# jcasal-homer/HomerHEVC

Measured on AMD Instinct MI355X. Metric: encoded frames/sec, 1080p & 2160p YUV420 fixed-QP IPPP, 1/2/4/8 MI355X, higher is better.
Workload: dtype int16; 1 GPU; cfg2-1080p-encode; sequences_per_gpu=256, width=1920, height=1080, wfpp_num_threads=17, qp=32, gop=IPPP intra_period=100

## Files before the change

homerhevc_amd/csrc/enc/enc_common.h:

```cpp
#pragma once
#include "enc_prims.h"
#if !defined(__HIPCC__)
#include <stdio.h>
#include <stdlib.h>
#endif

#if !defined(__HIPCC__) && defined(HENC_TRACE_ENABLE)
#include <stdio.h>
extern "C" FILE *henc_trace_file;
#define HENC_TRACE(...) do { if (henc_trace_file) fprintf(henc_trace_file, __VA_ARGS__); } while (0)
#define HENC_TRACE_PW(e, tag)                                                                                                                      \
	do {                                                                                                                                       \
		if (henc_trace_file) {                                                                                                             \
			unsigned a_[3] = {0, 0, 0};                                                                                                \
			for (int c_ = 0; c_ < 3; c_++) {                                                                                           \
				const int n_ = c_ ? 32 : 64;                                                                                       \
				const pred_t *p_ = c_ ? (e).w->pred_c[c_ - 1] : (e).w->pred_y;                                                     \
				for (int y_ = 0; y_ < n_; y_++)                                                                                    \
					for (int x_ = 0; x_ < n_; x_++) a_[c_] += (unsigned)(p_[y_ * n_ + x_] & 0xffff) * (unsigned)(1 + ((x_ + 3 * y_) & 7)); \
			}                                                                                                                          \
			fprintf(henc_trace_file, "PW %s ctu=%d pred=%u,%u,%u\n", tag, (e).ctu->ctu_number, a_[0], a_[1], a_[2]);                   \
		}                                                                                                                                  \
	} while (0)
#else
#define HENC_TRACE(...) do { } while (0)
#define HENC_TRACE_PW(e, tag) do { } while (0)
#endif

enum { PF_SETUP = 0, PF_MERGE, PF_ME_INT, PF_ME_SUB, PF_PRED_INTER, PF_ENC_INTER, PF_INTRA_SEARCH, PF_INTRA_TU, PF_INTRA_CHROMA, PF_CONSOLIDATE, PF_WAIT, PF_TOTAL, PF_PRIM0, PF_COUNT = PF_PRIM0 + 2 * PP_COUNT + 2 };
#if defined(__HIPCC__) && defined(HENC_PROFILE)
#define HENC_PROF_T0() const unsigned long long prof_t0_ = __builtin_amdgcn_s_memtime()
#if defined(HENC_QPROF)
#define HENC_PROF_ADD(e, cat) do { if ((cat) == PF_TOTAL && (e).prof && threadIdx.x == 0) (e).prof[cat] += __builtin_amdgcn_s_memtime() - prof_t0_; } while (0)
#define HENC_QPROF_T0() unsigned long long qprof_t_ = __builtin_amdgcn_s_memtime()
#define HENC_QPROF_MARK(e, cat) do { const unsigned long long now_ = __builtin_amdgcn_s_memtime(); if ((e).prof && threadIdx.x == 0) (e).prof[cat] += now_ - qprof_t_; qprof_t_ = now_; } while (0)
#define HENC_QPROF_ARG , unsigned long long &qprof_t_
#define HENC_QPROF_PASS , qprof_t_
#else
#define HENC_PROF_ADD(e, cat) do { if ((e).prof && threadIdx.x == 0) (e).prof[cat] += __builtin_amdgcn_s_memtime() - prof_t0_; } while (0)
#endif
#else
#define HENC_PROF_T0() do { } while (0)
#define HENC_PROF_ADD(e, cat) do { } while (0)
#endif
#if !defined(HENC_QPROF_MARK)
#define HENC_QPROF_T0() do { } while (0)
#define HENC_QPROF_MARK(e, cat) do { } while (0)
#define HENC_QPROF_ARG
#define HENC_QPROF_PASS
#endif

namespace henc {

#if defined(__HIPCC__)
extern __constant__ Geo henc_geo_table[NNODES];
#endif
#if defined(__HIP_DEVICE_COMPILE__)
struct GeoTable {
	const Geo *p;
	__device__ __forceinline__ const Geo &operator[](int i) const { return henc_geo_table[__builtin_amdgcn_readfirstlane(i)]; }
	__device__ __forceinline__ const Geo &lane(int i) const { return henc_geo_table[i]; }
};
#else
struct GeoTable {
	const Geo *p;
	HENC_INLINE const Geo &operator[](int i) const { return p[i]; }
	HENC_INLINE const Geo &lane(int i) const { return p[i]; }
};
#endif

constexpr int NHELP_MAX = 3;
constexpr int NODES_RESIDENT = 21, NODES_D3 = 85, NODE_QUAD_D3 = 16, NODE_QUAD_D4 = 64, NODE_SLOTS = NODES_RESIDENT + NODE_QUAD_D3 + NODE_QUAD_D4;
HENC_INLINE int node_quadrant(int idx) { return idx < NODES_D3 ? (idx - NODES_RESIDENT) >> 4 : (idx - NODES_D3) >> 6; }
HENC_INLINE int node_slot(int idx)
{
	return idx < NODES_RESIDENT ? idx : (idx < NODES_D3 ? NODES_RESIDENT + ((idx - NODES_RESIDENT) & (NODE_QUAD_D3 - 1)) : NODES_RESIDENT + NODE_QUAD_D3 + ((idx - NODES_D3) & (NODE_QUAD_D4 - 1)));
}
constexpr int NHELP_ = 1
#if defined(HENC_NHELP)
	+ (HENC_NHELP) - 1
#endif
	;
constexpr int HSCRATCH_ELEMS = 2048 + 144;
constexpr int LDS_OFF_WORK = 0, LDS_OFF_NODES = (int)((sizeof(Work) + 15) & ~(size_t)15), LDS_OFF_SEQ = LDS_OFF_NODES + (int)((sizeof(Node) * NODE_SLOTS + 15) & ~(size_t)15) + NHELP_ * HSCRATCH_ELEMS * 2,
	      LDS_OFF_FRAME = LDS_OFF_SEQ + (int)((sizeof(Seq) + 15) & ~(size_t)15), LDS_OFF_BOX = LDS_OFF_SEQ + (int)((sizeof(Seq) + sizeof(FrameCtx) + 31) & ~(size_t)15);
#if defined(__HIP_DEVICE_COMPILE__)
#define HENC_AT(T, OFFSET) LdsAt<T, OFFSET>
#else
#define HENC_AT(T, OFFSET) FastPtr<T>
#endif

constexpr int LDS_BOX_BYTES = 160, LDS_ENC_BYTES = 272;
constexpr int LDS_OFF_ENC = LDS_OFF_BOX + LDS_BOX_BYTES;
constexpr int LDS_OFF_RD = LDS_OFF_ENC + (1 + NHELP_) * LDS_ENC_BYTES;
struct Enc {
	unsigned long long *prof;
	HENC_AT(const Seq, LDS_OFF_SEQ) seq;
	HENC_AT(const FrameCtx, LDS_OFF_FRAME) f;
	const DevTables *T;
	FastPtr<const FastTables> ft;
	GeoTable geo;
	CtuInfo *ctus;
	CtuPublic *ctu;
// ... 450 lines not shown
```

homerhevc_amd/csrc/enc/enc_inter.h:

```cpp
#pragma once
#include "enc_common.h"

namespace henc {

#if !defined(__HIPCC__)
template <class G>
HENC_HD void mc_luma_interp(const G g, Enc &__restrict__ e, const int16_t *ref, int rs, int16_t *pred, int ps, int n, int mvx, int mvy)
{
	HENC_ENC_IN_LDS(e);
	const int xf = mvx & 3, yf = mvy & 3;
	const int16_t *src = ref + (mvy >> 2) * rs + (mvx >> 2);
	if (xf == 0) interp_stage<8>(g, src, rs, pred, ps, yf, n, n, 1, 1, 1);
	else if (yf == 0) interp_stage<8>(g, src, rs, pred, ps, xf, n, n, 0, 1, 1);
	else {
		int16_t *tmp = e.mc_tmp_y;
		const int ts = e.mc_tmp_y_stride;
		interp_stage<8>(g, src - 3 * rs, rs, tmp, ts, xf, n, n + 7, 0, 1, 0);
		interp_stage<8>(g, tmp + 3 * ts, ts, pred, ps, yf, n, n, 1, 0, 1);
	}
}
template <class G>
HENC_HD void mc_chroma_interp(const G g, Enc &__restrict__ e, const int16_t *ref, int rs, int16_t *pred, int ps, int n, int mvx, int mvy)
{
	HENC_ENC_IN_LDS(e);
// ... 86 lines not shown
}
template <int N>
HENC_INLINE uint32_t pick(const uint32_t (&a)[N], int idx)
{
#if defined(__HIP_DEVICE_COMPILE__)
	uint32_t v[N];
#pragma unroll
	for (int k = 0; k < N; k++) { v[k] = a[k]; asm("" : "+s"(v[k])); }
	uint32_t r = v[0];
#pragma unroll
	for (int k = 1; k < N; k++) r = idx == k ? v[k] : r;
	return r;
#else
	uint32_t r = a[0];
	for (int k = 1; k < N; k++) r = idx == k ? a[k] : r;
	return r;
#endif
}

HENC_INLINE uint32_t mv_cost_fast(const MvCandList &l, double corr, int mvx, int mvy, int *best_idx)
{
	uint32_t best = 0x7fffffff;
	int bi = 0;
	for (int i = 0; i < l.num; i++) {
		const double cx = corr * ((float)habs(l.mv[i].x - mvx)), cy = corr * ((float)habs(l.mv[i].y - mvy));
		const uint32_t c = (uint32_t)(cx + cy + .5);
		if (best > c) { best = c; bi = i; }
	}
	*best_idx = bi;
	return best;
}
HENC_INLINE float bit_sqrt(float x)
{
	union { float f; uint32_t u; } v;
	v.f = x;
	v.u += 127u << 23;
	v.u >>= 1;
	return v.f;
}
HENC_INLINE uint32_t mv_cost_sqrt(const MvCandList &l, uint32_t qp, int mvx, int mvy, int *best_idx)
{
	uint32_t best = 0x7fffffff;
	int bi = 0;
	for (int i = 0; i < l.num; i++) {
		const double cx = (float)qp * bit_sqrt((float)habs(l.mv[i].x - mvx));
		const double cy = (float)qp * bit_sqrt((float)habs(l.mv[i].y - mvy));
		const uint32_t c = (uint32_t)(3. + cx + cy + .5);
		if (best > c) { best = c; bi = i; }
	}
	*best_idx = bi;
	return best;
}

template <class G>
HENC_HD uint32_t motion_estimation(const G g, Enc &__restrict__ e, int ox, int oy, int gx, int gy, int size, const MvCandList &amvp, const MvCandList &search, double corr,
				   int action, MV *mv_io, MV *subpix_out)
{
	HENC_ENC_IN_LDS(e);
	static constexpr int ds[4][2] = {{-1, 0}, {0, -1}, {1, 0}, {0, 1}};
	static constexpr int db[8][2] = {{-2, 0}, {-1, -1}, {0, -2}, {1, -1}, {2, 0}, {1, 1}, {0, 2}, {-1, 1}};
	static constexpr int ref_h[9][2] = {{0, 0}, {0, -1}, {0, 1}, {-1, 0}, {1, 0}, {-1, -1}, {1, -1}, {-1, 1}, {1, 1}};
	static constexpr int ref_q[9][2] = {{0, 0}, {0, -1}, {0, 1}, {-1, -1}, {1, -1}, {-1, 0}, {1, 0}, {-1, 1}, {1, 1}};
	const int fw = e.seq->width, fh = e.seq->height;
	const int xlow = (gx - SEARCH_RANGE_X) < 0 ? -gx : -SEARCH_RANGE_X, xhigh = (gx + SEARCH_RANGE_X) > (fw - size) ? fw - gx - size : SEARCH_RANGE_X;
	const int ylow = (gy - SEARCH_RANGE_Y) < 0 ? -gy : -SEARCH_RANGE_Y, yhigh = (gy + SEARCH_RANGE_Y) > (fh - size) ? fh - gy - size : SEARCH_RANGE_Y;
	uint32_t cur_sad = 0, cur_rd = 0, best_sad = 0xffffffffu;
	int cur_x = 0, cur_y = 0, best_x = 0, best_y = 0, mvx = 0, mvy = 0, subx = 0, suby = 0, dummy;
#define HENC_IN_WIN(x, y) ((x) >= xlow && (x) <= xhigh && (y) >= ylow && (y) <= yhigh)
#define HENC_TRY(x, y, sad_, on_better)                                                            \
	do {                                                                                       \
		if (HENC_IN_WIN(x, y)) {                                                           \
			const uint32_t s_ = (sad_);                                                \
			const uint32_t rd_ = s_ + mv_cost_fast(amvp, corr, (x) << 2, (y) << 2, &dummy); \
			if (rd_ < cur_rd) { on_better; cur_sad = s_; cur_rd = rd_; cur_x = (x); cur_y = (y); } \
		}                                                                                  \
	} while (0)
	HENC_PROF_T0();
	if (action & ME_PEL) {
		bool early = false;
		cur_x = hclip(0, xlow, xhigh);
		cur_y = hclip(0, ylow, yhigh);
		{
			int qx[4], qy[4];
			bool ok[4];
			uint32_t s4[4];
			qx[0] = cur_x << 2; qy[0] = cur_y << 2; ok[0] = true;
			for (int i = 0; i < 3; i++) {
				const int x = i < search.num ? search.mv[i].x >> 2 : 0, y = i < search.num ? search.mv[i].y >> 2 : 0;
				qx[i + 1] = x << 2; qy[i + 1] = y << 2;
				ok[i + 1] = i < search.num && !(x == 0 && y == 0) && HENC_IN_WIN(x, y);
			}
			cand_sads<4>(g, e, ox, oy, gx, gy, size, qx, qy, ok, s4);
			cur_sad = s4[0];
			cur_rd = cur_sad + mv_cost_fast(amvp, corr, cur_x << 2, cur_y << 2, &dummy);
			best_sad = cur_sad; best_x = cur_x; best_y = cur_y;
			if (best_sad <= 0) early = true;
			if (!early) {
				for (int i = 0; i < search.num; i++) {
					const int x = search.mv[i].x >> 2, y = search.mv[i].y >> 2;
					if (x == 0 && y == 0) continue;
					HENC_TRY(x, y, pick(s4, i + 1), (void)0);
				}
				best_sad = cur_sad; best_x = cur_x; best_y = cur_y;
				if (best_sad <= 0) early = true;
			}
		}
// ... 46 lines not shown
				}
				cand_sads<4>(g, e, ox, oy, gx, gy, size, qx, qy, ok, s4);
				for (int i = next_start; i < next_start + search_size; i++) {
					const int idx = i % 4, x = best_x + ds[idx][0], y = best_y + ds[idx][1];
					HENC_TRY(x, y, pick(s4, idx), (next_start = (idx - 1 + 4) % 4, search_size = 3));
				}
				if (best_x == cur_x && best_y == cur_y) break;
				best_sad = cur_sad; best_x = cur_x; best_y = cur_y;
			}
		}
		best_sad = cur_sad; best_x = cur_x; best_y = cur_y;
		mvx = best_x << 2; mvy = best_y << 2;
	} else {
		mvx = mv_io->x; mvy = mv_io->y;
	}
	HENC_PROF_ADD(e, PF_ME_INT);
	if (action & ME_HALF) {
		int bidx = 0, bx = 0, by = 0;
		best_x = mvx >> 2; best_y = mvy >> 2;
		int qx[9], qy[9];
		bool ok[9];
		uint32_t sads[9];
		for (int i = 0; i < 9; i++) { qx[i] = (best_x << 2) + ref_h[i][0] * 2; qy[i] = (best_y << 2) + ref_h[i][1] * 2; ok[i] = true; }
		cand_sads<9>(g, e, ox, oy, gx, gy, size, qx, qy, ok, sads);
		if (!(action & ME_PEL)) cur_sad = sads[0];
		for (int i = 0; i < 9; i++) {
			const int cx = ref_h[i][0] * 2, cy = ref_h[i][1] * 2;
			const uint32_t s = pick(sads, i);
			if (s < cur_sad) { cur_sad = s; bx = cx; by = cy; bidx = i; }
		}
		mvx = (best_x << 2) + bx; mvy = (best_y << 2) + by; subx = bx; suby = by;
		best_sad = cur_sad;
		if (action & ME_QUARTER) {
			const int hx = ref_h[bidx][0], hy = ref_h[bidx][1];
			bx = hx * 2; by = hy * 2;
			for (int i = 0; i < 9; i++) { qx[i] = (best_x << 2) + hx * 2 + ref_q[i][0]; qy[i] = (best_y << 2) + hy * 2 + ref_q[i][1]; }
			cand_sads<9>(g, e, ox, oy, gx, gy, size, qx, qy, ok, sads);
			for (int i = 0; i < 9; i++) {
				const int cx = hx * 2 + ref_q[i][0], cy = hy * 2 + ref_q[i][1];
				const uint32_t s = pick(sads, i);
				if (s < cur_sad) { cur_sad = s; bx = cx; by = cy; }
			}
			best_sad = cur_sad;
			mvx = (best_x << 2) + bx; mvy = (best_y << 2) + by; subx = bx; suby = by;
		}
	}
#undef HENC_IN_WIN
#undef HENC_TRY
	HENC_PROF_ADD(e, PF_ME_SUB);
	mv_io->x = mvx; mv_io->y = mvy;
	subpix_out->x = subx; subpix_out->y = suby;
	return best_sad;
}

struct CornerNodes { int lb, tl, tr; };
HENC_INLINE CornerNodes corner_nodes(Enc &__restrict__ e, int ni)
{
	HENC_ENC_IN_LDS(e);
	const Geo &q = e.geo[ni];
	const int np = q.size >> 2, base = cfg_depth_start(CFG_MAX_CU_DEPTH);
	CornerNodes c;
	c.lb = base + raster2abs(q.raster_index + 16 * (np - 1));
	c.tl = base + raster2abs(q.raster_index);
	c.tr = base + raster2abs(q.raster_index + np - 1);
	return c;
}
struct NbUnit {
	int there, pred_mode, inter_mode, ref_idx;
	MV mv;
};
HENC_INLINE NbUnit nb_unit(Enc &__restrict__ e, const CtuPublic *c, uint32_t idx)
{
	HENC_ENC_IN_LDS(e);
	const CtuPublic *p = c ? c : e.ctu;
	const uint32_t i = c ? idx : 0;
	NbUnit u;
	u.pred_mode = p->pred_mode[i];
	u.inter_mode = p->inter_mode[i];
	u.ref_idx = p->mv_ref_idx[i];
	u.mv = p->mv_ref[i];
	u.there = c != nullptr;
	return u;
}
HENC_INLINE int equal_motion(const NbUnit &a, const NbUnit &b)
{
	if (a.inter_mode != b.inter_mode) return 0;
	if (a.inter_mode & 1) {
		if (a.mv.x != b.mv.x || a.mv.y != b.mv.y || a.ref_idx != b.ref_idx) return 0;
	}
	return 1;
}

HENC_INLINE int add_amvp_cand(MvCandList &l, const NbUnit &u)
{
	if (u.there && u.ref_idx >= 0) {
		l.mv[l.num++] = u.mv;
		return 1;
	}
	return 0;
}
HENC_INLINE void get_amvp_candidates(Enc &__restrict__ e, int ni, MvCandList &l)
{
	HENC_ENC_IN_LDS(e);
	const CornerNodes cn = corner_nodes(e, ni);
	uint32_t idx_lb = 0, idx_l = 0, idx_tr = 0, idx_t = 0, idx_tl = 0;
	l.num = 0;
// ... 475 lines not shown
```

homerhevc_amd/csrc/k_primtest.hip:

```cpp
#include <stdlib.h>
#include <string.h>
#include <vector>

#include "common.h"
#include "enc/enc_prims.h"

using namespace henc;

hmr_gpu_ctx *hmr_default_ctx();

namespace {

enum { PT_SAD = 1, PT_SSD, PT_PREDICT, PT_RECONST, PT_VARIANCE, PT_INTRA_PRED, PT_FILL_REFS, PT_ADI_FILTER, PT_TRANSFORM, PT_ITRANSFORM, PT_QUANT, PT_INV_QUANT };

struct PtArgs {
	int op, bytes;
	int p[12];
	long off[6];
};

int g_bytes = 0;

__global__ __launch_bounds__(64) void k_primtest(PtArgs a, int16_t *arena, uint8_t *arena8, const DevTables *T, uint32_t *ret)
{
	const WaveGrp g{(int)threadIdx.x};
	const int *p = a.p;
	auto A = [&](int k) { return arena + a.off[k]; };
	auto B = [&](int k) { return arena8 + a.off[k]; };
	uint32_t r = 0;
	switch (a.op) {
	case PT_SAD: r = blk_sad(g, A(0), p[0], A(1), p[1], p[2]); break;
	case PT_SSD: r = a.bytes ? blk_ssd(g, B(0), p[0], B(1), p[1], p[2]) : blk_ssd(g, A(0), p[0], A(1), p[1], p[2]); break;
	case PT_PREDICT:
		if (a.bytes) blk_predict(g, B(0), p[0], B(1), p[1], A(2), p[2], p[3]);
		else blk_predict(g, A(0), p[0], A(1), p[1], A(2), p[2], p[3]);
		break;
	case PT_RECONST: {
		const int16_t *res = p[1] ? A(1) : nullptr;
		if (a.bytes) blk_reconst(g, B(0), p[0], res, p[1], A(2), p[2], p[3]);
		else blk_reconst(g, A(0), p[0], res, p[1], A(2), p[2], p[3]);
		break;
	}
	case PT_VARIANCE: r = a.bytes ? blk_modified_variance(g, B(0), p[1], p[0], p[2]) : blk_modified_variance(g, A(0), p[1], p[0], p[2]); break;
	case PT_INTRA_PRED:
		if (a.bytes) {
			intra_predict(g, B(0), p[0], A(1), p[1], p[2], p[3]);
			g.sync();
			for (int i = g.tid; i < p[1] * p[1]; i += 64) A(0)[(i / p[1]) * p[0] + i % p[1]] = B(0)[(i / p[1]) * p[0] + i % p[1]];
		} else intra_predict(g, A(0), p[0], A(1), p[1], p[2], p[3]);
		break;
	case PT_FILL_REFS: intra_fill_refs(g, A(0), p[0], p[1], p[2], p[3], p[4], p[5], p[6], p[7], A(1)); break;
	case PT_ADI_FILTER: intra_adi_filter(g, A(0), A(1), p[0], p[1]); break;
	case PT_TRANSFORM:
		if (a.bytes) tr_forward(g, (const FastTables *)nullptr, T, B(0), p[0], B(3), p[0], A(1), A(2), p[1], p[2]);
		else tr_forward(g, (const FastTables *)nullptr, T, A(0), p[0], A(3), p[0], A(1), A(2), p[1], p[2]);
		break;
	case PT_ITRANSFORM: tr_inverse(g, (const FastTables *)nullptr, T, A(0), p[0], A(1), A(2), p[1], p[2]); break;
	case PT_QUANT: r = (uint32_t)quantize(g, (const FastTables *)nullptr, T, A(0), A(1), A(2), p[0], p[1], p[2], p[3], p[4], p[5], p[6], p[7], p[8]); break;
// ... 16 lines not shown
	if (!c) { fprintf(stderr, "hmr_gpu_prim_*: no device\n"); abort(); }
	PtArgs a;
	memset(&a, 0, sizeof a);
	a.op = op;
	a.bytes = g_bytes;
	for (int i = 0; i < np; i++) a.p[i] = p[i];
	size_t total = 0;
	for (int k = 0; k < nops; k++) {
		a.off[k] = (long)total;
		total += (ops[k].elems + 31) & ~(size_t)31;
	}
	std::vector<int16_t> h(total, 0);
	std::vector<uint8_t> h8(total, 0);
	for (int k = 0; k < nops; k++)
		if (ops[k].in) memcpy(h.data() + a.off[k], ops[k].in, ops[k].elems * 2);
	for (size_t i = 0; i < total; i++) h8[i] = (uint8_t)h[i];
	int16_t *d = nullptr;
	uint8_t *d8 = nullptr;
	uint32_t *dr = nullptr, r = 0;
	if (hipMalloc((void **)&d, total * 2 + 64) != hipSuccess || hipMalloc((void **)&d8, total + 64) != hipSuccess || hipMalloc((void **)&dr, 4) != hipSuccess) abort();
	(void)hipMemcpy(d, h.data(), total * 2, hipMemcpyHostToDevice);
	(void)hipMemcpy(d8, h8.data(), total, hipMemcpyHostToDevice);
	hipLaunchKernelGGL(k_primtest, dim3(1), dim3(64), 0, c->stream, a, d, d8, (const DevTables *)c->tables, dr);
	if (hipStreamSynchronize(c->stream) != hipSuccess) { fprintf(stderr, "hmr_gpu_prim_*: %s\n", hipGetErrorString(hipGetLastError())); abort(); }
	(void)hipMemcpy(h.data(), d, total * 2, hipMemcpyDeviceToHost);
	(void)hipMemcpy(&r, dr, 4, hipMemcpyDeviceToHost);
	for (int k = 0; k < nops; k++)
		if (ops[k].out) memcpy(ops[k].out, h.data() + a.off[k], ops[k].elems * 2);
	(void)hipFree(d); (void)hipFree(d8); (void)hipFree(dr);
	return r;
}

template <int MAXC>
__device__ __forceinline__ void multi_sad_all(const WaveGrp g, const uint8_t *src, const uint8_t *plane, const long long *off, int stride, int n, uint32_t *out)
{
	const uint8_t *cand[MAXC];
#pragma unroll
	for (int k = 0; k < MAXC; k++) cand[k] = off[k] < 0 ? nullptr : plane + off[k];
	uint32_t r[MAXC];
	multi_sad_u8<MAXC>(g, src, n, cand, stride, r);
	if (g.tid == 0) {
#pragma unroll
		for (int k = 0; k < MAXC; k++) out[k] = r[k];
	}
}
__global__ __launch_bounds__(64) void k_primtest_multi_sad(int maxc, const uint8_t *src, const uint8_t *plane, const long long *off, int stride, int n, uint32_t *out)
{
	const WaveGrp g{(int)threadIdx.x};
	off += (size_t)blockIdx.x * maxc;
	out += (size_t)blockIdx.x * maxc;
	if (maxc == 4) multi_sad_all<4>(g, src, plane, off, stride, n, out);
	else if (maxc == 8) multi_sad_all<8>(g, src, plane, off, stride, n, out);
	else multi_sad_all<9>(g, src, plane, off, stride, n, out);
}

size_t span(int stride, int rows, int cols) { return stride ? (size_t)stride * (rows - 1) + cols : (size_t)cols; }

}

extern "C" {

void hmr_gpu_prim_bytes(int on) { g_bytes = on ? 1 : 0; }

uint32_t hmr_gpu_prim_sad(int16_t *src, uint32_t src_stride, int16_t *pred, uint32_t pred_stride, int size)
{
	if (g_bytes) {
		std::vector<uint8_t> blk(64 * 64, 0), plane(span((int)pred_stride, size, size));
		for (int y = 0; y < size; y++)
			for (int x = 0; x < size; x++) {
				blk[y * 64 + x] = (uint8_t)src[(size_t)y * src_stride + x];
				plane[(size_t)y * pred_stride + x] = (uint8_t)pred[(size_t)y * pred_stride + x];
			}
		const int64_t off[4] = {0, -1, 0, -1};
		uint32_t out[4] = {0, 0, 0, 0};
		if (hmr_gpu_prim_multi_sad(4, blk.data(), plane.data(), plane.size(), off, 1, (int)pred_stride, size, out) != HMR_GPU_OK) { fprintf(stderr, "hmr_gpu_prim_sad: %s\n", hmr_gpu_last_error()); return 0xFFFFFFFFu; }
		if (out[1] != 0 || out[3] != 0 || out[2] != out[0]) {
			hmr_set_error("hmr_gpu_prim_sad: candidates {p, -, p, -} gave %u %u %u %u", out[0], out[1], out[2], out[3]);
			fprintf(stderr, "%s\n", hmr_gpu_last_error());
			return 0xFFFFFFFFu;
		}
		return out[0];
	}
	Operand ops[2] = {{src, nullptr, span((int)src_stride, size, size)}, {pred, nullptr, span((int)pred_stride, size, size)}};
	const int p[3] = {(int)src_stride, (int)pred_stride, size};
	return run(PT_SAD, p, 3, ops, 2);
}
uint32_t hmr_gpu_prim_ssd16b(int16_t *src, uint32_t src_stride, int16_t *pred, uint32_t pred_stride, int size)
{
	Operand ops[2] = {{src, nullptr, span((int)src_stride, size, size)}, {pred, nullptr, span((int)pred_stride, size, size)}};
	const int p[3] = {(int)src_stride, (int)pred_stride, size};
	return run(PT_SSD, p, 3, ops, 2);
}
void hmr_gpu_prim_predict(int16_t *orig, int orig_stride, int16_t *pred, int pred_stride, int16_t *residual, int residual_stride, int size)
{
	Operand ops[3] = {{orig, nullptr, span(orig_stride, size, size)}, {pred, nullptr, span(pred_stride, size, size)}, {residual, residual, span(residual_stride, size, size)}};
	const int p[4] = {orig_stride, pred_stride, residual_stride, size};
	run(PT_PREDICT, p, 4, ops, 3);
}
void hmr_gpu_prim_reconst(int16_t *pred, int pred_stride, int16_t *residual, int residual_stride, int16_t *decoded, int decoded_stride, int size)
{
	Operand ops[3] = {{pred, nullptr, span(pred_stride, size, size)}, {residual, nullptr, span(residual_stride, size, size)}, {decoded, decoded, span(decoded_stride, size, size)}};
	const int p[4] = {pred_stride, residual_stride, decoded_stride, size};
	run(PT_RECONST, p, 4, ops, 3);
}
uint32_t hmr_gpu_prim_modified_variance(int16_t *ptr, int size, int stride, int modif)
{
// ... 50 lines not shown
	const int p[3] = {block_stride, n, is_dst};
	run(PT_ITRANSFORM, p, 3, ops, 3);
}
void hmr_gpu_prim_quant(int16_t *src, int16_t *dst, int16_t *delta_u, int scan_mode, int depth, int comp, int is_intra, int slice_is_intra, int sign_hiding, int *ac_sum,
			int cu_size, int per, int rem)
{
	Operand ops[3] = {{src, nullptr, (size_t)cu_size * cu_size}, {nullptr, dst, (size_t)cu_size * cu_size}, {nullptr, delta_u, (size_t)cu_size * cu_size}};
	const int p[9] = {scan_mode, depth, comp, is_intra, slice_is_intra, sign_hiding, cu_size, per, rem};
	*ac_sum = (int)run(PT_QUANT, p, 9, ops, 3);
}
void hmr_gpu_prim_inv_quant(int16_t *src, int16_t *dst, int depth, int comp, int is_intra, int cu_size, int per, int rem)
{
	Operand ops[2] = {{src, nullptr, (size_t)cu_size * cu_size}, {nullptr, dst, (size_t)cu_size * cu_size}};
	const int p[6] = {depth, comp, is_intra, cu_size, per, rem};
	run(PT_INV_QUANT, p, 6, ops, 2);
}
int hmr_gpu_prim_multi_sad(int maxc, const uint8_t *src, const uint8_t *plane, size_t plane_bytes, const int64_t *cand_off, int ncalls, int stride, int n, uint32_t *out)
{
	if (!src || !plane || !cand_off || !out || ncalls < 1 || ncalls > 65536 || (maxc != 4 && maxc != 8 && maxc != 9) || (n != 8 && n != 16 && n != 32 && n != 64) || stride < 1) {
		hmr_set_error("hmr_gpu_prim_multi_sad: maxc 4 / 8 / 9, n 8 / 16 / 32 / 64, a stride of at least 1, 1 .. 65536 lists");
		return HMR_GPU_ERR_ARG;
	}
	for (int i = 0; i < ncalls * maxc; i++) {
		const int64_t o = cand_off[i];
		if (o == -1) continue;
		if (o < 0 || (uint64_t)o + (uint64_t)(n - 1) * (uint64_t)stride + (uint64_t)n > (uint64_t)plane_bytes) {
			hmr_set_error("hmr_gpu_prim_multi_sad: candidate %d of list %d does not lie inside the plane", i % maxc, i / maxc);
			return HMR_GPU_ERR_ARG;
		}
	}
	hmr_gpu_ctx *c = hmr_default_ctx();
	if (!c) { hmr_set_error("hmr_gpu_prim_multi_sad: no device"); return HMR_GPU_ERR_NO_DEVICE; }
	HIP_TRY(hipSetDevice(c->device));
	struct Bufs {
		void *p[4] = {nullptr, nullptr, nullptr, nullptr};
		~Bufs() { for (void *q : p) if (q) (void)hipFree(q); }
	} b;
	const size_t nres = (size_t)ncalls * maxc;
	HIP_TRY(hipMalloc(&b.p[0], 64 * 64));
	HIP_TRY(hipMalloc(&b.p[1], plane_bytes));
	HIP_TRY(hipMalloc(&b.p[2], nres * 8));
	HIP_TRY(hipMalloc(&b.p[3], nres * 4));
	HIP_TRY(hipMemsetAsync(b.p[0], 0, 64 * 64, c->stream));
	HIP_TRY(hipMemcpyAsync(b.p[0], src, (size_t)64 * n, hipMemcpyHostToDevice, c->stream));
	HIP_TRY(hipMemcpyAsync(b.p[1], plane, plane_bytes, hipMemcpyHostToDevice, c->stream));
	HIP_TRY(hipMemcpyAsync(b.p[2], cand_off, nres * 8, hipMemcpyHostToDevice, c->stream));
	hipLaunchKernelGGL(k_primtest_multi_sad, dim3(ncalls), dim3(64), 0, c->stream, maxc, (const uint8_t *)b.p[0], (const uint8_t *)b.p[1], (const long long *)b.p[2], stride, n, (uint32_t *)b.p[3]);
	HIP_TRY(hipGetLastError());
	HIP_TRY(hipMemcpyAsync(out, b.p[3], nres * 4, hipMemcpyDeviceToHost, c->stream));
	HIP_TRY(hipStreamSynchronize(c->stream));
	return HMR_GPU_OK;
}

}
```

include/homer_gpu.h:

```cpp
#ifndef HOMER_GPU_H
#define HOMER_GPU_H

#include <stddef.h>
#include <stdint.h>

#ifdef __cplusplus
extern "C" {
#endif

typedef struct hmr_gpu_ctx hmr_gpu_ctx;

enum hmr_gpu_status {
	HMR_GPU_OK = 0,
	HMR_GPU_ERR_NO_DEVICE = -1,
	HMR_GPU_ERR_HIP = -2,
	HMR_GPU_ERR_ARG = -3,
	HMR_GPU_ERR_NOMEM = -4
};


int hmr_gpu_create(hmr_gpu_ctx **out, int device, void *stream);
void hmr_gpu_destroy(hmr_gpu_ctx *ctx);
const char *hmr_gpu_last_error(void);
int hmr_gpu_sync(hmr_gpu_ctx *ctx);
// ... 409 lines not shown
int hmr_gpu_ssim(const int64_t sums[3], int width, int height, double ssim[3]);
int hmr_gpu_ssim_host(const hmr_gpu_picture *a, const hmr_gpu_picture *b, int width, int height, int64_t sums[3]);

int hmr_gpu_enc_export_pictures_rgb_device(hmr_gpu_enc **encs, int n, const int *which, const hmr_gpu_rgb_picture *outs, const hmr_gpu_rgb_picture *refs, uint64_t *dev_ssd,
					   void *consumer_stream);
int hmr_gpu_enc_export_picture_rgb_device(hmr_gpu_enc *enc, int which, const hmr_gpu_rgb_picture *out, const hmr_gpu_rgb_picture *ref, uint64_t *dev_ssd, void *consumer_stream);
int hmr_gpu_rgb_from_yuv_host(const uint8_t *y, const uint8_t *u, const uint8_t *v, int width, int height, const hmr_gpu_rgb_picture *out);
int hmr_gpu_rgb_ssd_host(const hmr_gpu_rgb_picture *a, const hmr_gpu_rgb_picture *b, int width, int height, uint64_t ssd[3]);
int hmr_gpu_psnr_rgb(const uint64_t ssd[3], int width, int height, double psnr[4]);

typedef struct hmr_gpu_scaled_rgb_picture {
	hmr_gpu_rgb_picture pic;
	int32_t width, height;
} hmr_gpu_scaled_rgb_picture;
int hmr_gpu_enc_load_sources_scaled_rgb_device(hmr_gpu_enc **encs, int n, const int *slots, const hmr_gpu_scaled_rgb_picture *pics, void *producer_stream);
int hmr_gpu_enc_load_source_scaled_rgb_device(hmr_gpu_enc *enc, int slot, const hmr_gpu_scaled_rgb_picture *pic, void *producer_stream);
int hmr_gpu_scale_rgb_host(const hmr_gpu_scaled_rgb_picture *pic, int dst_w, int dst_h, uint8_t *y, uint8_t *u, uint8_t *v);

enum { HMR_GPU_YUV_PLANAR = 0, HMR_GPU_YUV_SEMIPLANAR = 1, HMR_GPU_YUV_PACKED422 = 2 };
enum { HMR_GPU_CHROMA_420 = 0, HMR_GPU_CHROMA_422 = 1, HMR_GPU_CHROMA_444 = 2 };
typedef struct hmr_gpu_yuv_picture {
	int32_t format, chroma, bits, msb_aligned;
	int32_t offset[3], reserved;
	const void *plane[3];
	int64_t pitch[3];
} hmr_gpu_yuv_picture;
int hmr_gpu_yuv_picture_check(const hmr_gpu_yuv_picture *pic, int width, int height);
int hmr_gpu_yuv_convert_host(const hmr_gpu_yuv_picture *pic, int width, int height, uint8_t *y, uint8_t *u, uint8_t *v);
int hmr_gpu_enc_load_source_yuv_device(hmr_gpu_enc *enc, int slot, const hmr_gpu_yuv_picture *pic, void *producer_stream);
int hmr_gpu_enc_load_sources_yuv_device(hmr_gpu_enc **encs, int n, const int *slots, const hmr_gpu_yuv_picture *pics, void *producer_stream);

int hmr_gpu_subpel_planes(hmr_gpu_ctx *ctx, const int16_t *pic_y, const int16_t *pic_u, const int16_t *pic_v, int stride_y, int rows_y, int stride_c, int rows_c,
			  uint8_t *out_y, uint8_t *out_u, uint8_t *out_v);

int hmr_gpu_probe_valu_issue(hmr_gpu_ctx *ctx, int waves_per_simd, int dependent, double *wave_instr_per_s, double *ms);
int hmr_gpu_probe_issue(hmr_gpu_ctx *ctx, int op, int waves_per_simd, int dependent, double *wave_instr_per_s, double *ms);

void hmr_gpu_prim_bytes(int on);
uint32_t hmr_gpu_prim_sad(int16_t *src, uint32_t src_stride, int16_t *pred, uint32_t pred_stride, int size);
uint32_t hmr_gpu_prim_ssd16b(int16_t *src, uint32_t src_stride, int16_t *pred, uint32_t pred_stride, int size);
void hmr_gpu_prim_predict(int16_t *orig, int orig_stride, int16_t *pred, int pred_stride, int16_t *residual, int residual_stride, int size);
void hmr_gpu_prim_reconst(int16_t *pred, int pred_stride, int16_t *residual, int residual_stride, int16_t *decoded, int decoded_stride, int size);
uint32_t hmr_gpu_prim_modified_variance(int16_t *p, int size, int stride, int modif);
void hmr_gpu_prim_intra_planar(int16_t *prediction, int pred_stride, int16_t *adi_pred_buff, int adi_size, int cu_size);
void hmr_gpu_prim_intra_angular(int16_t *prediction, int pred_stride, int16_t *adi_pred_buff, int adi_size, int cu_size, int cu_mode, int is_luma);
void hmr_gpu_prim_fill_reference_samples(int16_t *decoded_corner, int stride, int n, int left, int top, int bottom_left, int top_right, int bl_size, int tr_size, int16_t *adi);
void hmr_gpu_prim_adi_filter(int16_t *adi, int16_t *out, int adi_size, int n, int strong_enabled);
void hmr_gpu_prim_transform(int16_t *block, int16_t *coeff, int block_stride, int n, int is_dst);
void hmr_gpu_prim_itransform(int16_t *block, int16_t *coeff, int block_stride, int n, int is_dst);
void hmr_gpu_prim_quant(int16_t *src, int16_t *dst, int16_t *delta_u, int scan_mode, int depth, int comp, int is_intra, int slice_is_intra, int sign_hiding, int *ac_sum,
			int cu_size, int per, int rem);
void hmr_gpu_prim_inv_quant(int16_t *src, int16_t *dst, int depth, int comp, int is_intra, int cu_size, int per, int rem);
int hmr_gpu_prim_multi_sad(int maxc, const uint8_t *src, const uint8_t *plane, size_t plane_bytes, const int64_t *cand_off, int ncalls, int stride, int n, uint32_t *out);

enum hmr_gpu_walk_step { HMR_GPU_WALK_QUAD8_Y = 1, HMR_GPU_WALK_QUAD8_C, HMR_GPU_WALK_QUAD16_Y, HMR_GPU_WALK_QUAD16_C, HMR_GPU_WALK_TU, HMR_GPU_WALK_TU_PAIR };
typedef struct hmr_gpu_walk_case {
	int32_t step, node, comp, one_slot;
	int32_t qp, ctu_x, ctu_y, slice_type;
	int32_t sign_hiding, chroma_qp_offset, stride_y, stride_c;
	int32_t mv[4][2];
	double avg_dist, chroma_weight;
	int64_t sub_y, sub_c[2], curr, pred;
} hmr_gpu_walk_case;
typedef struct hmr_gpu_walk_out {
	uint32_t dist[4][3];
	int32_t sum[4][3];
	uint32_t raw[4][3], cbf[4][3];
	uint32_t stray, reserved[15];
	uint8_t pred[4][256];
	int16_t rec[4][256], lv[4][256];
} hmr_gpu_walk_out;
int hmr_gpu_walk_forms(const hmr_gpu_walk_case *cases, int ncases, const uint8_t *arena, size_t arena_bytes, hmr_gpu_walk_out *out);

#ifdef __cplusplus
}
#endif
#endif
```

Baseline: 490.4 frames/s.

## Evaluate motion-search candidates lane-parallel with wave-wide SAD rounds on device

```diff
diff --git a/homerhevc_amd/csrc/enc/enc_common.h b/homerhevc_amd/csrc/enc/enc_common.h
--- a/homerhevc_amd/csrc/enc/enc_common.h
+++ b/homerhevc_amd/csrc/enc/enc_common.h
@@ -33,7 +33,14 @@
 #if defined(HENC_QPROF)
 #define HENC_PROF_ADD(e, cat) do { if ((cat) == PF_TOTAL && (e).prof && threadIdx.x == 0) (e).prof[cat] += __builtin_amdgcn_s_memtime() - prof_t0_; } while (0)
 #define HENC_QPROF_T0() unsigned long long qprof_t_ = __builtin_amdgcn_s_memtime()
+#if defined(HENC_QPROF_ME)
+#define HENC_QPROF_MARK(e, cat) do { (void)qprof_t_; } while (0)
+#define HENC_MEPROF_T0() unsigned long long meprof_t_ = __builtin_amdgcn_s_memtime()
+#define HENC_MEPROF_MARK(e, cat) do { const unsigned long long now_ = __builtin_amdgcn_s_memtime(); if ((e).prof && threadIdx.x == 0) (e).prof[cat] += now_ - meprof_t_; meprof_t_ = now_; } while (0)
+#define HENC_MEPROF_COUNT(e, cat) do { if ((e).prof && threadIdx.x == 0) (e).prof[cat] += 1; } while (0)
+#else
 #define HENC_QPROF_MARK(e, cat) do { const unsigned long long now_ = __builtin_amdgcn_s_memtime(); if ((e).prof && threadIdx.x == 0) (e).prof[cat] += now_ - qprof_t_; qprof_t_ = now_; } while (0)
+#endif
 #define HENC_QPROF_ARG , unsigned long long &qprof_t_
 #define HENC_QPROF_PASS , qprof_t_
 #else
@@ -49,6 +56,12 @@
 #define HENC_QPROF_ARG
 #define HENC_QPROF_PASS
 #endif
+#if !defined(HENC_MEPROF_MARK)
+#define HENC_MEPROF_T0() do { } while (0)
+#define HENC_MEPROF_MARK(e, cat) do { } while (0)
+#define HENC_MEPROF_COUNT(e, cat) do { } while (0)
+#endif
+enum { ME_MARK_SETUP = 1, ME_MARK_SADS, ME_MARK_WALK_INT, ME_MARK_WALK_SUB, ME_MARK_REST, ME_COUNT_SEARCHES, ME_COUNT_ROUNDS };
 
 namespace henc {
 
diff --git a/homerhevc_amd/csrc/enc/enc_inter.h b/homerhevc_amd/csrc/enc/enc_inter.h
--- a/homerhevc_amd/csrc/enc/enc_inter.h
+++ b/homerhevc_amd/csrc/enc/enc_inter.h
@@ -162,6 +162,206 @@
 	return best;
 }
 
+#if defined(__HIPCC__)
+struct MeAmvp { int num, x0, y0, x1, y1; };
+__device__ __forceinline__ uint32_t lane_mv_cost(const MeAmvp &a, double corr, int mvx, int mvy)
+{
+	uint32_t best = 0x7fffffff;
+	{
+		const double cx = corr * ((float)habs(a.x0 - mvx)), cy = corr * ((float)habs(a.y0 - mvy));
+		const uint32_t c = (uint32_t)(cx + cy + .5);
+		best = (a.num > 0 && best > c) ? c : best;
+	}
+	{
+		const double cx = corr * ((float)habs(a.x1 - mvx)), cy = corr * ((float)habs(a.y1 - mvy));
+		const uint32_t c = (uint32_t)(cx + cy + .5);
+		best = (a.num > 1 && best > c) ? c : best;
+	}
+	return best;
+}
+__device__ __forceinline__ int me_nibble(uint32_t packed, int k) { return (int)(packed << (28 - 4 * k)) >> 28; }
+#if defined(HENC_QPROF_ME)
+#define HENC_MEPROF_ARG , unsigned long long &meprof_t_
+#define HENC_MEPROF_PASS , meprof_t_
+#else
+#define HENC_MEPROF_ARG
+#define HENC_MEPROF_PASS
+#endif
+template <int MAXC, class G>
+__device__ __forceinline__ void lane_round_sads(const G g, Enc &__restrict__ e, int ox, int oy, int gx, int gy, int size, int vqx, int vqy, bool vok, uint32_t (&out)[MAXC] HENC_MEPROF_ARG)
+{
+	const uint64_t okm = __ballot(vok);
+	int qx[MAXC], qy[MAXC];
+	bool ok[MAXC];
+#pragma unroll
+	for (int k = 0; k < MAXC; k++) {
+		qx[k] = __builtin_amdgcn_readlane(vqx, k);
+		qy[k] = __builtin_amdgcn_readlane(vqy, k);
+		ok[k] = (okm >> k) & 1;
+	}
+	HENC_MEPROF_MARK(e, ME_MARK_SETUP);
+	cand_sads<MAXC>(g, e, ox, oy, gx, gy, size, qx, qy, ok, out);
+	HENC_MEPROF_MARK(e, ME_MARK_SADS);
+	HENC_MEPROF_COUNT(e, ME_COUNT_ROUNDS);
+}
+template <int MAXC, class G>
+__device__ __forceinline__ void lane_round(const G g, Enc &__restrict__ e, int ox, int oy, int gx, int gy, int size, int vx, int vy, bool vok, uint32_t vcost, uint32_t &vsad, uint32_t &vrd HENC_MEPROF_ARG)
+{
+	uint32_t s[MAXC];
+	lane_round_sads<MAXC>(g, e, ox, oy, gx, gy, size, vx << 2, vy << 2, vok, s HENC_MEPROF_PASS);
+	const int lane = g.tid;
+	uint32_t vs = 0;
+#pragma unroll
+	for (int k = 0; k < MAXC; k++) {
+		asm("" : "+s"(s[k]));
+		vs = lane == k ? s[k] : vs;
+	}
+	vsad = vs;
+	vrd = vok ? vs + vcost : 0xffffffffu;
+}
+template <class G>
+HENC_HD uint32_t motion_estimation(const G g, Enc &__restrict__ e, int ox, int oy, int gx, int gy, int size, const MvCandList &amvp, const MvCandList &search, double corr,
+				   int action, MV *mv_io, MV *subpix_out)
+{
+	HENC_ENC_IN_LDS(e);
+	const int lane = g.tid;
+	const int fw = e.seq->width, fh = e.seq->height;
+	const int xlow = (gx - SEARCH_RANGE_X) < 0 ? -gx : -SEARCH_RANGE_X, xhigh = (gx + SEARCH_RANGE_X) > (fw - size) ? fw - gx - size : SEARCH_RANGE_X;
+	const int ylow = (gy - SEARCH_RANGE_Y) < 0 ? -gy : -SEARCH_RANGE_Y, yhigh = (gy + SEARCH_RANGE_Y) > (fh - size) ? fh - gy - size : SEARCH_RANGE_Y;
+	uint32_t cur_sad = 0, cur_rd = 0, best_sad = 0xffffffffu;
+	int cur_x = 0, cur_y = 0, best_x = 0, best_y = 0, mvx = 0, mvy = 0, subx = 0, suby = 0;
+#define HENC_IN_WIN(x, y) ((x) >= xlow && (x) <= xhigh && (y) >= ylow && (y) <= yhigh)
+#define HENC_LANE(v, k) __builtin_amdgcn_readlane((int)(v), (k))
+#define HENC_TAKE(k)                                                                                                     \
+	do {                                                                                                             \
+		if ((k) >= 0) { cur_sad = (uint32_t)HENC_LANE(vsad, k); cur_x = HENC_LANE(x, k); cur_y = HENC_LANE(y, k); } \
+	} while (0)
+	HENC_PROF_T0();
+	HENC_MEPROF_T0();
+	HENC_MEPROF_COUNT(e, ME_COUNT_SEARCHES);
+	if (action & ME_PEL) {
+		const MeAmvp a = {uni(amvp.num), uni(amvp.mv[0].x), uni(amvp.mv[0].y), uni(amvp.mv[1].x), uni(amvp.mv[1].y)};
+		const int ds_x = (lane & 1) ? 0 : (lane & 3) - 1, ds_y = (lane & 1) ? (lane & 3) - 2 : 0;
+		const int db_x = me_nibble(0xF01210FEu, lane & 7), db_y = me_nibble(0x1210FEF0u, lane & 7);
+		bool early = false;
+		cur_x = hclip(0, xlow, xhigh);
+		cur_y = hclip(0, ylow, yhigh);
+		{
+			const int snum = uni(search.num), si = hclip(lane - 1, 0, 2);
+			const bool pred = lane >= 1 && lane - 1 < snum;
+			const int x = lane == 0 ? cur_x : (pred ? search.mv[si].x >> 2 : 0), y = lane == 0 ? cur_y : (pred ? search.mv[si].y >> 2 : 0);
+			const bool vok = lane == 0 || (pred && !(x == 0 && y == 0) && HENC_IN_WIN(x, y));
+			uint32_t vsad, vrd;
+			lane_round<4>(g, e, ox, oy, gx, gy, size, x, y, vok, lane_mv_cost(a, corr, x << 2, y << 2), vsad, vrd HENC_MEPROF_PASS);
+			cur_sad = (uint32_t)HENC_LANE(vsad, 0);
+			cur_rd = (uint32_t)HENC_LANE(vrd, 0);
+			best_sad = cur_sad; best_x = cur_x; best_y = cur_y;
+			if (best_sad <= 0) early = true;
+			if (!early) {
+				int ck = -1;
+#pragma unroll
+				for (int i = 1; i < 4; i++) {
+					const uint32_t rd = (uint32_t)HENC_LANE(vrd, i);
+					if (rd < cur_rd) { cur_rd = rd; ck = i; }
+				}
+				HENC_TAKE(ck);
+				best_sad = cur_sad; best_x = cur_x; best_y = cur_y;
+				if (best_sad <= 0) early = true;
+			}
+			HENC_MEPROF_MARK(e, ME_MARK_WALK_INT);
+		}
+		if (!early) {
+			const int x = best_x + ds_x, y = best_y + ds_y;
+			uint32_t vsad, vrd;
+			lane_round<4>(g, e, ox, oy, gx, gy, size, x, y, HENC_IN_WIN(x, y), lane_mv_cost(a, corr, x << 2, y << 2), vsad, vrd HENC_MEPROF_PASS);
+			int ck = -1;
+#pragma unroll
+			for (int i = 0; i < 4; i++) {
+				const uint32_t rd = (uint32_t)HENC_LANE(vrd, i);
+				if (rd < cur_rd) { cur_rd = rd; ck = i; }
+			}
+			HENC_TAKE(ck);
+			HENC_MEPROF_MARK(e, ME_MARK_WALK_INT);
+			if (best_sad <= 0) early = true;
+		}
+		if (!early) {
+			int dist = 2;
+			const int end = (best_x != 0 && best_y != 0) ? 4 : 8;
+			int next_start = 0, search_size = 8;
+			best_sad = cur_sad; best_x = cur_x; best_y = cur_y;
+			while (dist < end) {
+				const int x = best_x + db_x * dist, y = best_y + db_y * dist;
+				uint32_t vsad, vrd;
+				lane_round<8>(g, e, ox, oy, gx, gy, size, x, y, HENC_IN_WIN(x, y), lane_mv_cost(a, corr, x << 2, y << 2), vsad, vrd HENC_MEPROF_PASS);
+				int ck = -1;
+				for (int i = next_start; i < next_start + search_size; i++) {
+					const int idx = i & 7;
+					const uint32_t rd = (uint32_t)HENC_LANE(vrd, idx);
+					if (rd < cur_rd) { next_start = (idx - 2 + 8) & 7; search_size = 5; cur_rd = rd; ck = idx; }
+				}
+				HENC_TAKE(ck);
+				HENC_MEPROF_MARK(e, ME_MARK_WALK_INT);
+				dist *= 2;
+			}
+		}
+		best_sad = cur_sad; best_x = cur_x; best_y = cur_y;
+		{
+			int next_start = 0, search_size = 4;
+			for (;;) {
+				const int x = best_x + ds_x, y = best_y + ds_y;
+				uint32_t vsad, vrd;
+				lane_round<4>(g, e, ox, oy, gx, gy, size, x, y, HENC_IN_WIN(x, y), lane_mv_cost(a, corr, x << 2, y << 2), vsad, vrd HENC_MEPROF_PASS);
+				int ck = -1;
+				for (int i = next_start; i < next_start + search_size; i++) {
+					const int idx = i & 3;
+					const uint32_t rd = (uint32_t)HENC_LANE(vrd, idx);
+					if (rd < cur_rd) { next_start = (idx - 1 + 4) & 3; search_size = 3; cur_rd = rd; ck = idx; }
+				}
+				HENC_TAKE(ck);
+				HENC_MEPROF_MARK(e, ME_MARK_WALK_INT);
+				if (best_x == cur_x && best_y == cur_y) break;
+				best_sad = cur_sad; best_x = cur_x; best_y = cur_y;
+			}
+		}
+		best_sad = cur_sad; best_x = cur_x; best_y = cur_y;
+		mvx = best_x << 2; mvy = best_y << 2;
+	} else {
+		mvx = mv_io->x; mvy = mv_io->y;
+	}
+	HENC_MEPROF_MARK(e, ME_MARK_REST);
+	HENC_PROF_ADD(e, PF_ME_INT);
+	if (action & ME_HALF) {
+		const int rx = me_nibble(0x1F1F1F00u, lane & 7), ry_h = me_nibble(0x11FF001Fu, lane & 7), ry_q = me_nibble(0x1100FF1Fu, lane & 7);
+		const int last = (action & ME_QUARTER) ? 2 : 1;
+		int offx = 0, offy = 0;
+		best_x = mvx >> 2; best_y = mvy >> 2;
+		for (int stage = (action & ME_PEL) ? 1 : 0; stage <= last; stage++) {
+			const int dx = stage == 0 ? 0 : (stage == 1 ? rx * 2 : offx + rx), dy = stage == 0 ? 0 : (stage == 1 ? ry_h * 2 : offy + ry_q);
+			uint32_t s[8];
+			lane_round_sads<8>(g, e, ox, oy, gx, gy, size, (best_x << 2) + dx, (best_y << 2) + dy, stage != 0 || lane == 0, s HENC_MEPROF_PASS);
+			if (stage == 0) cur_sad = s[0];
+			else {
+				int bk = -1;
+#pragma unroll
+				for (int k = 0; k < 8; k++)
+					if (s[k] < cur_sad) { cur_sad = s[k]; bk = k; }
+				if (bk >= 0) { offx = HENC_LANE(dx, bk); offy = HENC_LANE(dy, bk); }
+			}
+			HENC_MEPROF_MARK(e, ME_MARK_WALK_SUB);
+		}
+		mvx = (best_x << 2) + offx; mvy = (best_y << 2) + offy; subx = offx; suby = offy;
+		best_sad = cur_sad;
+	}
+#undef HENC_IN_WIN
+#undef HENC_LANE
+#undef HENC_TAKE
+	HENC_MEPROF_MARK(e, ME_MARK_REST);
+	HENC_PROF_ADD(e, PF_ME_SUB);
+	mv_io->x = mvx; mv_io->y = mvy;
+	subpix_out->x = subx; subpix_out->y = suby;
+	return best_sad;
+}
+#else
 template <class G>
 HENC_HD uint32_t motion_estimation(const G g, Enc &__restrict__ e, int ox, int oy, int gx, int gy, int size, const MvCandList &amvp, const MvCandList &search, double corr,
 				   int action, MV *mv_io, MV *subpix_out)
@@ -314,6 +514,7 @@
 	subpix_out->x = subx; subpix_out->y = suby;
 	return best_sad;
 }
+#endif
 
 struct CornerNodes { int lb, tl, tr; };
 HENC_INLINE CornerNodes corner_nodes(Enc &__restrict__ e, int ni)
diff --git a/homerhevc_amd/csrc/k_primtest.hip b/homerhevc_amd/csrc/k_primtest.hip
--- a/homerhevc_amd/csrc/k_primtest.hip
+++ b/homerhevc_amd/csrc/k_primtest.hip
@@ -3,7 +3,7 @@
 #include <vector>
 
 #include "common.h"
-#include "enc/enc_prims.h"
+#include "enc/enc_inter.h"
 
 using namespace henc;
 
@@ -126,6 +126,44 @@
 	if (maxc == 4) multi_sad_all<4>(g, src, plane, off, stride, n, out);
 	else if (maxc == 8) multi_sad_all<8>(g, src, plane, off, stride, n, out);
 	else multi_sad_all<9>(g, src, plane, off, stride, n, out);
+}
+
+constexpr unsigned ME_LDS_BYTES = LDS_OFF_ENC + LDS_ENC_BYTES;
+static_assert(sizeof(hmr_gpu_prim_me_case) == 80 && sizeof(hmr_gpu_prim_me_out) == 20, "include/homer_gpu.h section 15 states these layouts");
+__global__ __launch_bounds__(64) void k_primtest_motion_search(const hmr_gpu_prim_me_case *cases, const uint8_t *src, const uint8_t *plane0, int size, int stride, int width, int height,
+							       hmr_gpu_prim_me_out *out)
+{
+	extern __shared__ __align__(16) uint8_t lds[];
+	const WaveGrp g{(int)threadIdx.x};
+	const hmr_gpu_prim_me_case &cs = cases[blockIdx.x];
+	for (int i = g.tid; i < (int)(ME_LDS_BYTES / 4); i += 64) ((uint32_t *)lds)[i] = 0;
+	g.sync();
+	Work *lw = (Work *)(lds + LDS_OFF_WORK);
+	Seq *lseq = (Seq *)(lds + LDS_OFF_SEQ);
+	FrameCtx *lframe = (FrameCtx *)(lds + LDS_OFF_FRAME);
+	const uint8_t *blk = src + (size_t)blockIdx.x * size * size;
+	for (int i = g.tid; i < size * size; i += 64) lw->curr_y[(i / size) * 64 + i % size] = blk[i];
+	if (g.tid == 0) {
+		lseq->width = width;
+		lseq->height = height;
+		lseq->stride_y = stride;
+		lframe->sub_y = plane0;
+		lw->amvp.num = cs.n_amvp;
+		for (int i = 0; i < 2; i++) { lw->amvp.mv[i].x = cs.amvp[i][0]; lw->amvp.mv[i].y = cs.amvp[i][1]; }
+		lw->search_cands.num = cs.n_search;
+		for (int i = 0; i < 3; i++) { lw->search_cands.mv[i].x = cs.search[i][0]; lw->search_cands.mv[i].y = cs.search[i][1]; }
+	}
+	g.sync();
+	Enc &e = *(Enc *)(lds + LDS_OFF_ENC);
+	HENC_ENC_IN_LDS(e);
+	MV mv = {cs.start[0], cs.start[1]}, subpix = {0, 0};
+	const uint32_t sad = motion_estimation(g, e, 0, 0, uni(cs.gx), uni(cs.gy), size, lw->amvp, lw->search_cands, cs.corr, uni(cs.action), &mv, &subpix);
+	if (g.tid == 0) {
+		hmr_gpu_prim_me_out &o = out[blockIdx.x];
+		o.mv[0] = mv.x; o.mv[1] = mv.y;
+		o.subpix[0] = subpix.x; o.subpix[1] = subpix.y;
+		o.sad = sad;
+	}
 }
 
 size_t span(int stride, int rows, int cols) { return stride ? (size_t)stride * (rows - 1) + cols : (size_t)cols; }
@@ -282,4 +320,58 @@
 	return HMR_GPU_OK;
 }
 
-}
+int hmr_gpu_prim_motion_search(const hmr_gpu_prim_me_case *cases, int ncases, int size, const uint8_t *src, const uint8_t *planes, size_t plane_bytes, int64_t origin, int stride,
+			       int width, int height, hmr_gpu_prim_me_out *out)
+{
+	if (!cases || !src || !planes || !out || ncases < 1 || ncases > 65536 || (size != 8 && size != 16 && size != 32 && size != 64) || width < size || height < size || width > 8192 ||
+	    height > 8192 || stride < width || stride > (1 << 16)) {
+		hmr_set_error("hmr_gpu_prim_motion_search: size 8 / 16 / 32 / 64, a picture of size .. 8192 samples each way, a stride of width .. 65536, 1 .. 65536 cases");
+		return HMR_GPU_ERR_ARG;
+	}
+	if (origin - 16 * (int64_t)stride - 1 < 0 || (uint64_t)origin + ((uint64_t)height * 16 + 15) * (uint64_t)stride + (uint64_t)width + 1 > (uint64_t)plane_bytes) {
+		hmr_set_error("hmr_gpu_prim_motion_search: the planes do not hold the picture with one sample around it");
+		return HMR_GPU_ERR_ARG;
+	}
+	auto vec_ok = [](const int32_t *v) { return v[0] >= -32768 && v[0] <= 32767 && v[1] >= -32768 && v[1] <= 32767; };
+	for (int i = 0; i < ncases; i++) {
+		const hmr_gpu_prim_me_case &k = cases[i];
+		bool ok = k.gx >= 0 && k.gx <= width - size && k.gy >= 0 && k.gy <= height - size && k.n_amvp >= 0 && k.n_amvp <= 2 && k.n_search >= 0 && k.n_search <= 3 && k.action >= 1 &&
+			  k.action <= 7 && k.corr >= 0. && k.corr <= 1e6 && vec_ok(k.amvp[0]) && vec_ok(k.amvp[1]) && vec_ok(k.search[0]) && vec_ok(k.search[1]) && vec_ok(k.search[2]) &&
+			  vec_ok(k.start);
+		if (ok && !(k.action & ME_PEL)) {
+			const int xlow = (k.gx - SEARCH_RANGE_X) < 0 ? -k.gx : -SEARCH_RANGE_X, xhigh = (k.gx + SEARCH_RANGE_X) > (width - size) ? width - k.gx - size : SEARCH_RANGE_X;
+			const int ylow = (k.gy - SEARCH_RANGE_Y) < 0 ? -k.gy : -SEARCH_RANGE_Y, yhigh = (k.gy + SEARCH_RANGE_Y) > (height - size) ? height - k.gy - size : SEARCH_RANGE_Y;
+			const int x = k.start[0] >> 2, y = k.start[1] >> 2;
+			ok = x >= xlow && x <= xhigh && y >= ylow && y <= yhigh;
+		}
+		if (!ok) {
+			hmr_set_error("hmr_gpu_prim_motion_search: case %d is outside the ranges of include/homer_gpu.h section 15", i);
+			return HMR_GPU_ERR_ARG;
+		}
+	}
+	hmr_gpu_ctx *c = hmr_default_ctx();
+	if (!c) { hmr_set_error("hmr_gpu_prim_motion_search: no device"); return HMR_GPU_ERR_NO_DEVICE; }
+	HIP_TRY(hipSetDevice(c->device));
+	HIP_TRY(hipFuncSetAttribute((const void *)k_primtest_motion_search, hipFuncAttributeMaxDynamicSharedMemorySize, (int)ME_LDS_BYTES));
+	struct Bufs {
+		void *p[4] = {nullptr, nullptr, nullptr, nullptr};
+		~Bufs() { for (void *q : p) if (q) (void)hipFree(q); }
+	} b;
+	const size_t case_bytes = sizeof(hmr_gpu_prim_me_case) * (size_t)ncases, src_bytes = (size_t)ncases * size * size, out_bytes = sizeof(hmr_gpu_prim_me_out) * (size_t)ncases;
+	HIP_TRY(hipMalloc(&b.p[0], case_bytes));
+	HIP_TRY(hipMalloc(&b.p[1], src_bytes));
+	HIP_TRY(hipMalloc(&b.p[2], plane_bytes));
+	HIP_TRY(hipMalloc(&b.p[3], out_bytes));
+	HIP_TRY(hipMemcpyAsync(b.p[0], cases, case_bytes, hipMemcpyHostToDevice, c->stream));
+	HIP_TRY(hipMemcpyAsync(b.p[1], src, src_bytes, hipMemcpyHostToDevice, c->stream));
+	HIP_TRY(hipMemcpyAsync(b.p[2], planes, plane_bytes, hipMemcpyHostToDevice, c->stream));
+	HIP_TRY(hipMemsetAsync(b.p[3], 0, out_bytes, c->stream));
+	hipLaunchKernelGGL(k_primtest_motion_search, dim3(ncases), dim3(64), ME_LDS_BYTES, c->stream, (const hmr_gpu_prim_me_case *)b.p[0], (const uint8_t *)b.p[1],
+			   (const uint8_t *)b.p[2] + origin, size, stride, width, height, (hmr_gpu_prim_me_out *)b.p[3]);
+	HIP_TRY(hipGetLastError());
+	HIP_TRY(hipMemcpyAsync(out, b.p[3], out_bytes, hipMemcpyDeviceToHost, c->stream));
+	HIP_TRY(hipStreamSynchronize(c->stream));
+	return HMR_GPU_OK;
+}
+
+}
diff --git a/include/homer_gpu.h b/include/homer_gpu.h
--- a/include/homer_gpu.h
+++ b/include/homer_gpu.h
@@ -485,6 +485,21 @@
 			int cu_size, int per, int rem);
 void hmr_gpu_prim_inv_quant(int16_t *src, int16_t *dst, int depth, int comp, int is_intra, int cu_size, int per, int rem);
 int hmr_gpu_prim_multi_sad(int maxc, const uint8_t *src, const uint8_t *plane, size_t plane_bytes, const int64_t *cand_off, int ncalls, int stride, int n, uint32_t *out);
+typedef struct hmr_gpu_prim_me_case {
+	int32_t gx, gy;
+	int32_t n_amvp, amvp[2][2];
+	int32_t n_search, search[3][2];
+	int32_t action;
+	int32_t start[2];
+	int32_t reserved;
+	double corr;
+} hmr_gpu_prim_me_case;
+typedef struct hmr_gpu_prim_me_out {
+	int32_t mv[2], subpix[2];
+	uint32_t sad;
+} hmr_gpu_prim_me_out;
+int hmr_gpu_prim_motion_search(const hmr_gpu_prim_me_case *cases, int ncases, int size, const uint8_t *src, const uint8_t *planes, size_t plane_bytes, int64_t origin, int stride,
+			       int width, int height, hmr_gpu_prim_me_out *out);
 
 enum hmr_gpu_walk_step { HMR_GPU_WALK_QUAD8_Y = 1, HMR_GPU_WALK_QUAD8_C, HMR_GPU_WALK_QUAD16_Y, HMR_GPU_WALK_QUAD16_C, HMR_GPU_WALK_TU, HMR_GPU_WALK_TU_PAIR };
 typedef struct hmr_gpu_walk_case {
```

New measurement: 499.1 frames/s (median of 6 runs). 1.8% higher.
